# SaurabhIndi/unet-segmentation

Measured on AMD Instinct MI355X. Metric: training images/sec (512×512×1, batch=8) at 1/2/4/8 MI355X; IoU vs ref, higher is better.
Workload: dtype fp32; 1 GPU; U-Net train step 512x512x1, batch 8/GPU, fp32 GEMMs (fwd+WCE+bwd+SGD); global_batch=8, image=512, parallelism=dp1

## Files before the change

include/unet_hip.h:

```cpp
#ifndef UNET_HIP_H
#define UNET_HIP_H

#include <stddef.h>
#include <stdint.h>

#ifdef __cplusplus
extern "C" {
#endif

typedef void* unet_stream_t;

const char* unet_version(void);
const char* unet_last_error(void);

typedef struct unet_plan unet_plan;

unet_plan* unet_plan_create(int n, int c_in, int h, int w, int n_classes);

enum { UNET_PREC_FP32 = 0, UNET_PREC_BF16 = 1, UNET_PREC_BF16X3 = 2 };
unet_plan* unet_plan_create_ex(int n, int c_in, int h, int w, int n_classes, int precision);
int unet_plan_precision(const unet_plan* p);
void unet_plan_destroy(unet_plan* p);
int unet_plan_out_hw(const unet_plan* p, int* out_h, int* out_w);
size_t unet_plan_workspace_bytes(const unet_plan* p);
// ... 72 lines not shown
size_t unet_instance_masks_ws_bytes(int n, int h, int w);
int unet_instance_masks(const uint8_t* mask, int n, int h, int w, int min_size, uint16_t* labels, void* ws,
                        unet_stream_t stream);
size_t unet_rand_index_ws_bytes(int h, int w);
int unet_rand_index(const uint16_t* gt, const uint16_t* pred, int h, int w, double* out, void* ws,
                    unet_stream_t stream);

typedef struct unet_tracker unet_tracker;
unet_tracker* unet_tracker_create(int h, int w, double iou_track, double iou_division, int max_children);
void unet_tracker_destroy(unet_tracker* t);
size_t unet_tracker_ws_bytes(int h, int w);
int unet_tracker_add_frame(unet_tracker* t, const uint16_t* labels, int frame, void* ws, unet_stream_t stream);
int unet_tracker_step_host(unet_tracker* t, int frame, int n_curr, const int32_t* host_labels,
                           const int64_t* host_areas, const int64_t* host_inter);
int unet_tracker_num_tracks(const unet_tracker* t);
int unet_tracker_tracks(const unet_tracker* t, int32_t* host_out, int cap);
int unet_linear_sum_assignment(long long nr, long long nc, const double* host_cost, int64_t* host_row_ind,
                               int64_t* host_col_ind);

enum { UNET_CTC_SEG = 0, UNET_CTC_TRA = 1 };
enum { UNET_CTC_GT = 0, UNET_CTC_RES = 1 };
typedef struct unet_ctc unet_ctc;
unet_ctc* unet_ctc_create(void);
void unet_ctc_destroy(unet_ctc* c);
size_t unet_ctc_ws_bytes(int t, int h, int w);
int unet_ctc_add_frames(unet_ctc* c, int kind, const uint16_t* gt, const uint16_t* res, const int32_t* host_frames,
                        int t, int h, int w, void* ws, unet_stream_t stream);
int unet_ctc_add_frame_host(unet_ctc* c, int kind, int frame, int n_gt, const int32_t* host_gt_labels,
                            const int64_t* host_gt_areas, int n_res, const int32_t* host_res_labels,
                            const int64_t* host_res_areas, int n_pairs, const int64_t* host_pairs);
int unet_ctc_set_tracks(unet_ctc* c, int side, const int32_t* host_rows, int n);
int unet_ctc_measures(unet_ctc* c, double* host_out, int64_t* host_counts);
long long unet_ctc_log(unet_ctc* c, char* buf, size_t cap);
int unet_ctc_num_frames(const unet_ctc* c, int kind);
int unet_ctc_frame_sizes(const unet_ctc* c, int kind, int index, int32_t* host_out);
int unet_ctc_frame_tables(const unet_ctc* c, int kind, int index, int32_t* host_gt_labels, int64_t* host_gt_areas,
                          int32_t* host_res_labels, int64_t* host_res_areas, int64_t* host_pairs);
int unet_ctc_stats(const unet_ctc* c, int64_t* host_out);

enum { UNET_WARP_FORCE_WS = 1 };
size_t unet_warping_error_ws_bytes(int n, int h, int w);
int unet_warping_error(const uint16_t* gt, const uint8_t* pred, int n, int h, int w, int radius, int separate,
                       int max_sweeps, int flags, uint8_t* warped, int64_t* counts, void* ws, unet_stream_t stream);
void unet_simple_point_table(uint8_t out[256]);

int unet_set_tuning(const char* key, int value);
size_t unet_tuning_report(char* buf, size_t len);
int unet_tuning_reset(void);
long long unet_slab_fallbacks(int reset);
long long unet_nondeterministic_sites(int reset);
long long unet_fused_bnb_sites(int reset);
long long unet_wgrad_oihw_sites(int reset);
long long unet_igemm_plane_launches(int reset);
int unet_tuning_save(const char* path);
int unet_tuning_load(const char* path);

int unet_conv3x3_fwd(const float* x, int n, int h, int w, int ci, const float* wt_oihw,
                     const float* bias, int co, const float* x_scale, const float* x_shift,
                     float* y, void* ws, unet_stream_t stream);
int unet_conv3x3_dgrad(const float* dy, int n, int h, int w, int ci, const float* wt_oihw,
                       int co, float* dx, void* ws, unet_stream_t stream);
int unet_conv3x3_wgrad(const float* x, const float* dy, int n, int h, int w, int ci, int co,
                       float* dw_oihw, float* db, void* ws, unet_stream_t stream);
size_t unet_conv_ws_bytes(int n, int h, int w, int ci, int co);
int unet_convT2_fwd(const float* x, int n, int h, int w, int ci, const float* wt, const float* bias,
                    int co, float* y, void* ws, unet_stream_t stream);
int unet_convT2_bwd(const float* x, const float* dy, int n, int h, int w, int ci, const float* wt,
                    int co, float* dx, float* dw, float* db, void* ws, unet_stream_t stream);
int unet_maxpool2_fwd(const float* x, int n, int h, int w, int c, float* y, uint8_t* arg,
                      unet_stream_t stream);
int unet_maxpool2_bwd(const float* dy, const uint8_t* arg, int n, int h, int w, int c, float* dx,
                      unet_stream_t stream);
int unet_bn_train_fwd(const float* x, int n, int h, int w, int c, const float* gamma,
                      const float* beta, float* running_mean, float* running_var, float* y,
                      float* save_mean, float* save_invstd, void* ws, unet_stream_t stream);
int unet_bn_train_bwd(const float* x, const float* dy, int n, int h, int w, int c,
                      const float* gamma, const float* save_mean, const float* save_invstd,
                      float* dx, float* dgamma, float* dbeta, void* ws, unet_stream_t stream);
size_t unet_bn_ws_bytes(int c);

size_t unet_bn_relu_ws_bytes(int n, int h, int w, int c);
int unet_bn_relu_fwd(const float* x, int n, int h, int w, int c, const float* gamma, const float* beta,
                     float* running_mean, float* running_var, int64_t* nbt, float momentum, float eps,
                     int training, int relu, float* y, float* save_mean, float* save_invstd, void* ws,
                     unet_stream_t stream);
int unet_bn_relu_bwd(const float* x, const float* y, const float* dy, int n, int h, int w, int c,
                     const float* gamma, const float* save_mean, const float* save_invstd, int training,
                     int relu, float* dx, float* dgamma, float* dbeta, void* ws, unet_stream_t stream);
size_t unet_conv_first_ws_bytes(int n, int ci, int h, int w);
int unet_conv_first_fwd(const float* x_nchw, int n, int ci, int h, int w, const float* wt, const float* bias,
                        float* y, unet_stream_t stream);
int unet_conv_first_bwd(const float* x_nchw, const float* dy, int n, int ci, int h, int w, const float* wt,
                        float* dx_nchw, float* dw, float* db, void* ws, unet_stream_t stream);
size_t unet_conv1x1_ws_bytes(int k);
int unet_conv1x1_fwd(const float* x, int n, int h, int w, int c, const float* wt, const float* bias, int k,
                     float* logits_nchw, unet_stream_t stream);
int unet_conv1x1_bwd(const float* x, const float* dlogits_nchw, int n, int h, int w, int c, const float* wt, int k,
                     float* dx, float* dw, float* db, void* ws, unet_stream_t stream);

int unet_peak_probe(int kind, int reps, double* result, unet_stream_t stream);

#ifdef __cplusplus
}
#endif
#endif
```

unet-segmentation_amd/csrc/ops.hip:

```cpp
#include <algorithm>
#include <cerrno>
#include <string>

#include "../../include/unet_hip.h"
#include "unet_internal.h"

using namespace unet;

namespace unet {
extern int g_tune_igemm, g_tune_wgrad, g_autotune, g_force_split, g_force_tile, g_concurrent, g_wino_max,
    g_wino_dgrad_max, g_wino_wgrad_max, g_bf16_norm, g_bn_fold, g_wino4_fwd_min_cg, g_wino4_fwd_small_cg,
    g_maxpool_vec8, g_wgrad_fwd_u, g_ctc_chunk_frames, g_ctc_dense_cells;
hipError_t launch_fill(float* p, size_t n, float v, hipStream_t s);
hipError_t launch_pair_sum(const double* st, int g, int c, float* out, hipStream_t s);
}

namespace {
thread_local std::string g_op_err;
inline size_t al256(size_t b) { return (b + 255) / 256 * 256; }
int g_op_prec = UNET_PREC_FP32;
int g_op_a16 = 0;

hipError_t op_b_to_bf16(IgemmArgs& a, size_t n, void* scratch, hipStream_t s) {
  if (g_op_prec == UNET_PREC_FP32) return hipSuccess;
// ... 482 lines not shown
                     const int64_t* ts, const int64_t* wsd, float* loss, float* dl, float gscale, void* ws,
                     unet_stream_t st) {
  if (!ts || !wsd || k < 1) return -EINVAL;
  OPCK(launch_wce(logits, t, wm, n, k, h, w, ts, wsd, loss, dl, gscale, reinterpret_cast<double*>(ws),
                  reinterpret_cast<hipStream_t>(st)));
  return 0;
}

int unet_scale_by_device_scalar(float* x, size_t n, const float* g, unet_stream_t st) {
  OPCK(launch_scale_by_dev(x, x, n, g, reinterpret_cast<hipStream_t>(st)));
  return 0;
}

int unet_scale_by_device_scalar_out(const float* x, float* y, size_t n, const float* g, unet_stream_t st) {
  OPCK(launch_scale_by_dev(x, y, n, g, reinterpret_cast<hipStream_t>(st)));
  return 0;
}

int unet_sgd_momentum(float* p, const float* g, float* buf, size_t n, float lr, float mom, float gscale, int first,
                      unet_stream_t st) {
  OPCK(launch_sgd(p, g, buf, n, lr, mom, gscale, first, reinterpret_cast<hipStream_t>(st)));
  return 0;
}

int unet_iou_counts(const uint8_t* a, const uint8_t* b, size_t n, unsigned long long* out, unet_stream_t st) {
  OPCK(launch_iou(a, b, n, out, reinterpret_cast<hipStream_t>(st)));
  return 0;
}

int unet_set_tuning(const char* key, int value) {
  if (!key) return -EINVAL;
  const std::string k(key);
  if (k == "igemm_variant") g_tune_igemm = value;
  else if (k == "wgrad_variant") g_tune_wgrad = value;
  else if (k == "autotune") g_autotune = value;
  else if (k == "force_split") g_force_split = value;
  else if (k == "force_tile") g_force_tile = value;
  else if (k == "concurrent") g_concurrent = value;
  else if (k == "wino_max") g_wino_max = value;
  else if (k == "bf16_norm") g_bf16_norm = value;
  else if (k == "bn_fold") g_bn_fold = value != 0;
  else if (k == "wino_dgrad_max") g_wino_dgrad_max = value;
  else if (k == "wino_wgrad_max") g_wino_wgrad_max = value;
  else if (k == "wino4_fwd_min_cg") g_wino4_fwd_min_cg = value;
  else if (k == "wino4_fwd_small_cg") g_wino4_fwd_small_cg = value;
  else if (k == "op_a16") g_op_a16 = value != 0;
  else if (k == "maxpool_vec8") g_maxpool_vec8 = value;
  else if (k == "bnb_fuse") g_bnb_fuse = value;
  else if (k == "wgrad_early_u") g_wgrad_early_u = value;
  else if (k == "wgrad_fwd_u") g_wgrad_fwd_u = value;
  else if (k == "wgrad_plane") g_wgrad_plane = value;
  else if (k == "wgrad_oihw") g_wgrad_oihw = value;
  else if (k == "igemm_plane") g_igemm_plane = value;
  else if (k == "wino_point_tile") g_wino_point_tile = value;
  else if (k == "ctc_chunk_frames" || k == "ctc_dense_cells") {
    if (value < -1 || (value == 0 && k == "ctc_chunk_frames")) return -EINVAL;
    (k == "ctc_chunk_frames" ? g_ctc_chunk_frames : g_ctc_dense_cells) = value;
  }
  else if (k == "deterministic") g_deterministic = value != 0;
  else if (k == "op_precision") {
    if (value != UNET_PREC_FP32 && value != UNET_PREC_BF16 && value != UNET_PREC_BF16X3) return -EINVAL;
    g_op_prec = value;
  } else return -EINVAL;
  return 0;
}

int unet_tile_gather(const float* image, int c, int h, int w, int tile_in, int tile_out, int top, int left, int nx,
                     int first, int stride, int ntiles, float* tiles, unet_stream_t st) {
  if (!image || !tiles) return -EINVAL;
  OPCK(launch_tile_gather(image, c, h, w, tile_in, tile_out, top, left, nx, first, stride, ntiles, tiles,
                          reinterpret_cast<hipStream_t>(st)));
  return 0;
}

int unet_tile_scatter(const float* tile_logits, int k, int tile_out, int nx, int first, int stride, int ntiles, int h,
                      int w, float* logits, uint8_t* mask, unet_stream_t st) {
  if (!tile_logits) return -EINVAL;
  OPCK(launch_tile_scatter(tile_logits, k, tile_out, nx, first, stride, ntiles, h, w, logits, mask,
                           reinterpret_cast<hipStream_t>(st)));
  return 0;
}

size_t unet_instance_masks_ws_bytes(int n, int h, int w) {
  return n > 0 && h > 0 && w > 0 ? instance_masks_ws_bytes(n, h, w) : 0;
}

int unet_instance_masks(const uint8_t* mask, int n, int h, int w, int min_size, uint16_t* labels, void* ws,
                        unet_stream_t st) {
  if (!mask || !labels || !ws) return -EINVAL;
  OPCK(launch_instance_masks(mask, n, h, w, min_size, labels, ws, reinterpret_cast<hipStream_t>(st)));
  return 0;
}

size_t unet_rand_index_ws_bytes(int h, int w) { return h > 0 && w > 0 ? rand_index_ws_bytes(h, w) : 0; }

int unet_rand_index(const uint16_t* gt, const uint16_t* pred, int h, int w, double* out, void* ws,
                    unet_stream_t st) {
  if (!gt || !pred || !out || !ws) return -EINVAL;
  OPCK(launch_rand_index(gt, pred, h, w, out, ws, reinterpret_cast<hipStream_t>(st)));
  return 0;
}

size_t unet_weight_map_ws_bytes(int n) { return n > 0 ? weight_map_ws_bytes(n) : 0; }

int unet_weight_map(const uint16_t* labels, int n, int h, int w, double w0, double sigma, float* weights,
                    double* weights64, void* ws, unet_stream_t st) {
// ... 51 lines not shown
```

unet-segmentation_amd/csrc/plan.hip:

```cpp
#include <cerrno>
#include <cstdio>
#include <cstdlib>
#include <cstring>
#include <algorithm>
#include <array>
#include <map>
#include <mutex>
#include <string>
#include <vector>

#include "../../include/unet_hip.h"
#include "unet_internal.h"

using namespace unet;

namespace unet {
extern int g_wino_max, g_wino_dgrad_max, g_wino_wgrad_max, g_wino4_fwd_min_cg, g_wino4_fwd_small_cg;
int g_autotune = getenv("UNET_AUTOTUNE") ? atoi(getenv("UNET_AUTOTUNE")) : 1;
int g_concurrent = getenv("UNET_CONCURRENT") ? atoi(getenv("UNET_CONCURRENT")) : 1;
int g_bf16_norm = getenv("UNET_BF16_NORM") ? atoi(getenv("UNET_BF16_NORM")) : 0;
int g_bn_fold = getenv("UNET_BN_FOLD") ? atoi(getenv("UNET_BN_FOLD")) : 1;
int g_force_split = 0;
int g_force_tile = 0;
int g_deterministic = getenv("UNET_DETERMINISTIC") ? atoi(getenv("UNET_DETERMINISTIC")) : 0;
// ... 1327 lines not shown
  CK(launch_conv_first_dgrad(dy0, p->n, p->cin, p->h, p->w, P<float>(prm, L.pw), dx, s));
  return 0;
}

int unet_plan_wait_segment(unet_plan* p, int seg, unet_stream_t stream) {
  if (!p || seg < 0 || seg >= 9) {
    set_err("unet_plan_wait_segment: bad argument");
    return -EINVAL;
  }
  if (!p->seg_on_side[seg] || !p->side) return 0;
  CK(hipStreamWaitEvent(reinterpret_cast<hipStream_t>(stream), p->ev_seg[seg], 0));
  return 0;
}

int unet_plan_join(unet_plan* p, unet_stream_t stream) {
  if (!p) {
    set_err("unet_plan_join: null plan");
    return -EINVAL;
  }
  if (!p->side || !p->side_pending) return 0;
  CK(hipEventRecord(p->ev_join, p->side));
  CK(hipStreamWaitEvent(reinterpret_cast<hipStream_t>(stream), p->ev_join, 0));
  p->side_pending = false;
  return 0;
}

size_t unet_tuning_report(char* buf, size_t len) {
  std::string r;
  {
    std::lock_guard<std::mutex> lk(g_tune_mu);
    for (const auto& kv : g_tune_log) r += kv.second + "\n";
  }
  if (buf && len > 0) {
    const size_t k = std::min(len - 1, r.size());
    memcpy(buf, r.data(), k);
    buf[k] = 0;
  }
  return r.size() + 1;
}

long long unet_nondeterministic_sites(int reset) {
  return reset ? g_nondet_sites.exchange(0) : g_nondet_sites.load();
}

long long unet_fused_bnb_sites(int reset) {
  return reset ? unet::g_fused_bnb_sites.exchange(0) : unet::g_fused_bnb_sites.load();
}
long long unet_wgrad_oihw_sites(int reset) {
  return reset ? unet::g_wgrad_oihw_sites.exchange(0) : unet::g_wgrad_oihw_sites.load();
}
long long unet_igemm_plane_launches(int reset) {
  return reset ? unet::g_igemm_plane_launches.exchange(0) : unet::g_igemm_plane_launches.load();
}
long long unet_slab_fallbacks(int reset) {
  return reset ? g_slab_fallbacks.exchange(0) : g_slab_fallbacks.load();
}

int unet_tuning_reset(void) {
  std::lock_guard<std::mutex> lk(g_tune_mu);
  g_tuned.clear();
  g_tune_log.clear();
  return 0;
}

int unet_tuning_save(const char* path) {
  if (!path) return -EINVAL;
  std::lock_guard<std::mutex> lk(g_tune_mu);
  FILE* f = fopen(path, "w");
  if (!f) return -errno;
  for (const auto& kv : g_tuned) fprintf(f, "%s\t%d\t%d\n", kv.first.c_str(), kv.second.tile, kv.second.split);
  fclose(f);
  return (int)g_tuned.size();
}

int unet_tuning_load(const char* path) {
  if (!path) return -EINVAL;
  std::lock_guard<std::mutex> lk(g_tune_mu);
  return tune_db_read(path, true);
}

int unet_plan_set_timing(unet_plan* p, int enable) {
  if (!p) return -EINVAL;
  p->timing = enable != 0;
  return 0;
}

int unet_plan_timing(const unet_plan* pc, double* ms, double* fl, double* by, int* cnt) {
  auto* p = const_cast<unet_plan*>(pc);
  if (!p) return -EINVAL;
  int rc = 0;
  for (auto& e : p->evs) {
    float t = 0;
    if (hipEventSynchronize(e.b) != hipSuccess || hipEventElapsedTime(&t, e.a, e.b) != hipSuccess) {
      set_err("unet_plan_timing: event query failed");
      rc = -EIO;
    } else {
      p->t_ms[e.cls] += t;
      p->t_fl[e.cls] += e.flops;
      p->t_by[e.cls] += e.bytes;
      p->t_xf[e.cls] += e.xflops;
      p->t_n[e.cls] += 1;
      if (e.site >= 0) {
        auto& v = p->sites[e.site];
        v[0] += t;
        v[1] += e.flops;
        v[2] += e.xflops;
// ... 45 lines not shown
```

unet-segmentation_amd/csrc/unet_internal.h:

```cpp
#pragma once
#include <hip/hip_runtime.h>
#include <cstddef>
#include <cstdint>
#include <atomic>
#include <string>
#include <vector>

namespace unet {

constexpr int kMaxInChannels = 4096;
constexpr int kMaxClassCount = 4096;

struct Src {
  const float* ptr = nullptr;
  int H = 0, W = 0, C = 0;
  int oy = 0, ox = 0;
  const float* scale = nullptr;
  const float* shift = nullptr;
  int h16 = 0;
};

struct Gather {
  Src s[2];
  int c_split = 0;
// ... 6 lines not shown

struct Dst {
  float* ptr = nullptr;
  int H = 0, W = 0, C = 0;
  int oy = 0, ox = 0;
  int h16 = 0;
};

struct Epilogue {
  const float* bias = nullptr;
  int shuffle_co = 0;
  Dst d[2];
  int n_split = 1 << 30;
  int relu = 0;
  double* stats = nullptr;
  const float* yref = nullptr;
  int yref_h16 = 0;
  const float* bn_scale = nullptr;
  const float* bn_shift = nullptr;
  const float* bn_mean = nullptr;
  const float* bn_invstd = nullptr;
  double* bstats = nullptr;
  double* colsum1 = nullptr;
};

constexpr int kStatGroups = 64;

struct IgemmArgs {
  Gather a;
  const float* b = nullptr;
  const uint16_t* bh = nullptr;
  const uint16_t* bl = nullptr;
  int M, N, K;
  Epilogue e;
  int ksplit = 1;
  float* slab = nullptr;
  float* wino_ws = nullptr;
  size_t wino_ws_bytes = 0;
  int batch = 1;
  int batch_rows = 0;
  long long batch_b = 0;
  struct { int tile = -1, split = 1; } wino_choice;
  int fwd = 0;
};

extern std::atomic<long long> g_slab_fallbacks;
extern int g_deterministic;
extern int g_bnb_fuse;
extern int g_wgrad_early_u;
extern int g_wgrad_plane;
extern int g_wgrad_oihw;
extern int g_igemm_plane;
extern std::atomic<long long> g_igemm_plane_launches;
extern int g_wino_point_tile;
extern std::atomic<long long> g_nondet_sites;

struct WgradArgs {
  Gather ga;
  Gather gb;
  int Mo, No;
  int P;
  int pix_per_split;
  float* out;
  float* out_oihw = nullptr;
  float* slab = nullptr;
  size_t slab_bytes = 0;
  int accumulate = 0;
  int bf16 = 0;
  int split = 0;
  int batch = 1;
  long long batch_a = 0, batch_b = 0, batch_out = 0;
  float* wino_ws = nullptr;
  size_t wino_ws_bytes = 0;
  const float* vd_pre = nullptr;
  int u_ready = 0;
  int abl = 0;
};

struct GemmChoice {
  int tile = -1;
  int split = 1;
};

enum class IgemmFamily {
  Reg,
  Halo,
  Conv3Dma,
  Ring,
  Flat,
  C64,
  GemmRing,
  Wino,
  WinoFused
};
struct IgemmTile {
  int id;
  IgemmFamily family;
  int bm, bn, bk, slots;
  int th, tw, ch;
  int wino_m;
  bool bf16;
  bool x3;
  bool ksplit;
  bool tuned;
  bool (*fits)(const IgemmArgs&, const IgemmTile&);
  hipError_t (*go)(const IgemmArgs&, hipStream_t);
// ... 223 lines not shown
```

unet-segmentation_amd/csrc/winograd.hip:

```cpp
#include <algorithm>
#include <cstdlib>

#include "gemm_common.h"
#include "ring_common.h"

namespace unet {

__global__ void k_wino_w(const float* __restrict__ b, int N, int Cg, float* __restrict__ v) {
  const long long i = blockIdx.x * (long long)blockDim.x + threadIdx.x;
  if (i >= (long long)N * Cg) return;
  const int n = (int)(i / Cg), c = (int)(i - (long long)n * Cg);
  float g[3][3];
#pragma unroll
  for (int t = 0; t < 9; ++t) g[t / 3][t % 3] = b[((size_t)n * 9 + t) * Cg + c];
  float tg[4][3];
#pragma unroll
  for (int k = 0; k < 3; ++k) {
    tg[0][k] = g[0][k];
    tg[1][k] = 0.5f * (g[0][k] + g[1][k] + g[2][k]);
    tg[2][k] = 0.5f * (g[0][k] - g[1][k] + g[2][k]);
    tg[3][k] = g[2][k];
  }
  const size_t plane = (size_t)N * Cg, o = (size_t)n * Cg + c;
#pragma unroll
// ... 1511 lines not shown
      acc[p] = __builtin_amdgcn_mfma_f32_16x16x4f32(b.y, a.y, acc[p], 0, 0, 0);
    }
    lgkm_wait0();
    raw_barrier();
    issue_v(kn, 1);
  }
  vm_wait<0>();
  __syncthreads();
  wf64_output(acc, g, e, N, T, Th, Tw, t0, n0, th, cb, mi, mq, lane, wave, lds);
}

bool wino_fused64p_applies(const IgemmArgs& a) { return wino_fused64_applies(a) && a.a.Cg <= kWf64pMaxCg; }

hipError_t launch_wino_fused64p(const IgemmArgs& a, hipStream_t s) {
  if (!wino_fused64p_applies(a)) return hipErrorInvalidValue;
  const Gather& g = a.a;
  const int Th = (g.Hg + 3) / 4, Tw = (g.Wg + 3) / 4;
  const long long T = (long long)g.nimg * Th * Tw;
  float* V = reinterpret_cast<float*>(a.wino_ws);
  const long long nw = (long long)a.N * g.Cg;
  const int NB = a.N / 64;
  const long long G = (T + 31) / 32 * NB;
  hipLaunchKernelGGL(k_wino4f_w8, dim3((unsigned)((nw + 255) / 256)), dim3(256), 0, s, a.b, a.N, g.Cg, V);
  hipLaunchKernelGGL(k_wino4f64p, dim3((unsigned)G), dim3(512), 0, s, g, (const float*)V, a.N, T, Th, Tw, NB, a.e);
  return hipGetLastError();
}

__global__ void k_wino2f_w8(const float* __restrict__ b, int N, int Cg, float* __restrict__ v) {
  const long long i = blockIdx.x * (long long)blockDim.x + threadIdx.x;
  if (i >= (long long)N * Cg) return;
  const int n = (int)(i / Cg), c = (int)(i - (long long)n * Cg);
  float g[3][3];
#pragma unroll
  for (int t = 0; t < 9; ++t) g[t / 3][t % 3] = b[((size_t)n * 9 + t) * Cg + c];
  float tg[4][3];
#pragma unroll
  for (int k = 0; k < 3; ++k) {
    tg[0][k] = g[0][k];
    tg[1][k] = 0.5f * (g[0][k] + g[1][k] + g[2][k]);
    tg[2][k] = 0.5f * (g[0][k] - g[1][k] + g[2][k]);
    tg[3][k] = g[2][k];
  }
  const size_t base = (size_t)(c >> 3) * 16 * N;
  const int pos = wf8_slot(n, c & 3) + ((c >> 2) & 1);
#pragma unroll
  for (int r = 0; r < 4; ++r) {
    const float w4[4] = {tg[r][0], 0.5f * (tg[r][0] + tg[r][1] + tg[r][2]), 0.5f * (tg[r][0] - tg[r][1] + tg[r][2]),
                         tg[r][2]};
#pragma unroll
    for (int q = 0; q < 4; ++q) v[(base + (size_t)(r * 4 + q) * N + n) * 8 + pos] = w4[q];
  }
}

template <int NC>
__global__ __launch_bounds__(512, NC == 32 ? 2 : 1) void k_wino2f64(Gather g, const float* __restrict__ V, int N,
                                                                   long long T, int Th, int Tw, int NB, Epilogue e) {
  constexpr int TT = 64;
  constexpr int PU = TT * 8;
  constexpr int PV = NC * 8;
  constexpr int NJ = NC / 32;
  __shared__ __attribute__((aligned(16))) float lds[16 * PU + 16 * PV];
  float* Us = lds;
  float* Vs = lds + 16 * PU;
  const int tid = threadIdx.x, lane = tid & 63, wave = tid >> 6;
  long long bid = blockIdx.x;
  const long long G = gridDim.x;
  if ((G & 7) == 0) bid = (bid & 7) * (G >> 3) + (bid >> 3);
  const int nb = (int)(bid % NB);
  const long long t0 = (bid / NB) * TT;
  const int n0 = nb * NC;

  const int lt = tid >> 3, lc = tid & 7;
  const long long t = t0 + lt;
  int img = 0, ty = 0, tx = 0;
  if (t < T) {
    tx = (int)(t % Tw);
    const long long r = t / Tw;
    ty = (int)(r % Th);
    img = (int)(r / Th);
  }
  const int vrows = t < T ? min(4, g.Hg + 2 - 2 * ty) : 0;
  const int vcols = t < T ? min(4, g.Wg + 2 - 2 * tx) : 0;
  const bool wfull = __all(vrows == 4 && vcols == 4);
  float* const ubase = Us + lt * 8 + wf8_slot(lt, lc & 3) + (lc >> 2);
  float raw[16];
  float sc = 1.f, sh = 0.f;
  const int nk = g.Cg >> 3;
  const unsigned long long vbase = uniform_u64(V);
  const unsigned vlds = (unsigned)(size_t)(lds_u8_t*)lds + (unsigned)(16 * PU * 4);
  auto load = [&](int kc) {
    const bool second = kc * 8 >= g.c_split;
    const float* sp = second ? g.s[1].ptr : g.s[0].ptr;
    const int sH = second ? g.s[1].H : g.s[0].H, sW = second ? g.s[1].W : g.s[0].W;
    const int sC = second ? g.s[1].C : g.s[0].C;
    const int soy = second ? g.s[1].oy : g.s[0].oy, sox = second ? g.s[1].ox : g.s[0].ox;
    const int cl = kc * 8 - (second ? g.c_split : 0) + lc;
    const float* scp = second ? g.s[1].scale : g.s[0].scale;
    if (scp) {
      sc = scp[cl];
      sh = (second ? g.s[1].shift : g.s[0].shift)[cl];
    }
    const char* sb = reinterpret_cast<const char*>(sp);
    const unsigned o0 = ((unsigned)((img * sH + 2 * ty + soy) * sW + 2 * tx + sox) * sC + cl) * 4u;
    const unsigned rs = (unsigned)sW * sC * 4u, cs = (unsigned)sC * 4u;
    if (wfull) {
#pragma unroll
      for (int yy = 0; yy < 4; ++yy)
#pragma unroll
        for (int xx = 0; xx < 4; ++xx)
          raw[yy * 4 + xx] = *reinterpret_cast<const float*>(sb + (o0 + (yy * rs + xx * cs)));
    } else {
      const unsigned lr = (unsigned)max(vrows - 1, 0), lcn = (unsigned)max(vcols - 1, 0);
#pragma unroll
      for (int yy = 0; yy < 4; ++yy)
#pragma unroll
        for (int xx = 0; xx < 4; ++xx)
          raw[yy * 4 + xx] = *reinterpret_cast<const float*>(
              sb + (o0 + (min((unsigned)yy, lr) * rs + min((unsigned)xx, lcn) * cs)));
    }
  };
  auto commit = [&](int kc) {
    const bool second = kc * 8 >= g.c_split;
    const float* scp = second ? g.s[1].scale : g.s[0].scale;
    __builtin_amdgcn_s_waitcnt(0x0F70);
#pragma unroll
    for (int j = 0; j < 2 * NJ; ++j) {
      const int pc = wave + 8 * j;
      dma_sv((unsigned)((((size_t)kc * 16 + pc / NJ) * N + n0) * 32) + (unsigned)((pc % NJ) * 1024 + lane * 16),
             vbase, vlds + (unsigned)((pc / NJ) * PV * 4 + (pc % NJ) * 1024));
    }
    if (scp) {
#pragma unroll
      for (int q = 0; q < 16; ++q) raw[q] = fmaxf(fmaf(raw[q], sc, sh), 0.f);
    }
    if (!wfull) {
#pragma unroll
      for (int q = 0; q < 16; ++q) raw[q] = (q / 4 < vrows && q % 4 < vcols) ? raw[q] : 0.f;
    }
    float ev[4][4];
#pragma unroll
    for (int xx = 0; xx < 4; ++xx) {
      ev[0][xx] = raw[0 * 4 + xx] - raw[2 * 4 + xx];
      ev[1][xx] = raw[1 * 4 + xx] + raw[2 * 4 + xx];
      ev[2][xx] = raw[2 * 4 + xx] - raw[1 * 4 + xx];
      ev[3][xx] = raw[1 * 4 + xx] - raw[3 * 4 + xx];
    }
#pragma unroll
    for (int a = 0; a < 4; ++a) {
      ubase[(a * 4 + 0) * PU] = ev[a][0] - ev[a][2];
      ubase[(a * 4 + 1) * PU] = ev[a][1] + ev[a][2];
      ubase[(a * 4 + 2) * PU] = ev[a][2] - ev[a][1];
      ubase[(a * 4 + 3) * PU] = ev[a][1] - ev[a][3];
    }
    vm_wait<0>();
  };

  const int th = wave & 3, ch = wave >> 2;
  const int mi = lane & 15, mq = lane >> 4;
  const int aoff = (16 * th + mi) * 8 + wf8_slot(16 * th + mi, mq);
  const int boff = (16 * NJ * ch + mi) * 8 + wf8_slot(mi, mq);
  floatx4 acc[16][NJ];
#pragma unroll
  for (int p = 0; p < 16; ++p)
#pragma unroll
    for (int j = 0; j < NJ; ++j) acc[p][j] = (floatx4){0.f, 0.f, 0.f, 0.f};
  load(0);
  for (int kc = 0; kc < nk; ++kc) {
    commit(kc);
    __syncthreads();
    if (kc + 1 < nk) load(kc + 1);
#pragma unroll
    for (int p = 0; p < 16; ++p) {
      const float2 a = *reinterpret_cast<const float2*>(Us + p * PU + aoff);
#pragma unroll
      for (int j = 0; j < NJ; ++j) {
        const float2 b = *reinterpret_cast<const float2*>(Vs + p * PV + boff + 16 * j * 8);
        acc[p][j] = __builtin_amdgcn_mfma_f32_16x16x4f32(b.x, a.x, acc[p][j], 0, 0, 0);
        acc[p][j] = __builtin_amdgcn_mfma_f32_16x16x4f32(b.y, a.y, acc[p][j], 0, 0, 0);
      }
    }
    __syncthreads();
  }

  const long long tt = t0 + 16 * th + mi;
  const bool want = e.stats || e.yref || e.colsum1;
  const int nsplit = e.n_split < N ? e.n_split : N;
  const int grp = blockIdx.x % kStatGroups;
#pragma unroll
  for (int j = 0; j < NJ; ++j) {
    const int col0 = n0 + 16 * NJ * ch + 16 * j + 4 * mq;
    const bool second = col0 >= e.n_split;
    float* dptr = second ? e.d[1].ptr : e.d[0].ptr;
    const int dC = second ? e.d[1].C : e.d[0].C;
    const int dcol = second ? col0 - e.n_split : col0;
    const bool bwd_mask = e.yref != nullptr && !second;
    const float4 bias = e.bias ? ld4(e.bias + col0) : make_float4(0.f, 0.f, 0.f, 0.f);
    float4 bsc = make_float4(0.f, 0.f, 0.f, 0.f), bsh = bsc, bmu = bsc, bis = bsc;
    if (bwd_mask) { bsc = ld4(e.bn_scale + col0); bsh = ld4(e.bn_shift + col0); bmu = ld4(e.bn_mean + col0); bis = ld4(e.bn_invstd + col0); }
    float s1[4] = {0.f, 0.f, 0.f, 0.f}, s2[4] = {0.f, 0.f, 0.f, 0.f};
    if (tt < T) {
      const int ox = (int)(tt % Tw);
      const long long rq = tt / Tw;
      const int oy = (int)(rq % Th), on = (int)(rq / Th);
      float4 y4[4];
      if (bwd_mask) {
#pragma unroll
        for (int a = 0; a < 2; ++a)
#pragma unroll
          for (int bb = 0; bb < 2; ++bb) {
            const int y = min(2 * oy + a, g.Hg - 1), x = min(2 * ox + bb, g.Wg - 1);
            y4[a * 2 + bb] = ld4(e.yref + ((size_t)(on * g.Hg + y) * g.Wg + x) * dC + dcol);
          }
      }
      __builtin_amdgcn_s_waitcnt(0x0F70);
      float o[4][2][2];
#pragma unroll
      for (int r = 0; r < 4; ++r) {
        float w[2][4];
#pragma unroll
        for (int xx = 0; xx < 4; ++xx) {
          const float m0 = acc[0 * 4 + xx][j][r], m1 = acc[1 * 4 + xx][j][r];
          const float m2 = acc[2 * 4 + xx][j][r], m3 = acc[3 * 4 + xx][j][r];
          w[0][xx] = m0 + m1 + m2;
          w[1][xx] = m1 - m2 - m3;
        }
#pragma unroll
        for (int a = 0; a < 2; ++a) {
          o[r][a][0] = w[a][0] + w[a][1] + w[a][2];
          o[r][a][1] = w[a][1] - w[a][2] - w[a][3];
        }
      }
      const float bsv[4] = {bias.x, bias.y, bias.z, bias.w};
      const float scv[4] = {bsc.x, bsc.y, bsc.z, bsc.w}, shv[4] = {bsh.x, bsh.y, bsh.z, bsh.w};
      const float muv[4] = {bmu.x, bmu.y, bmu.z, bmu.w}, isv[4] = {bis.x, bis.y, bis.z, bis.w};
#pragma unroll
      for (int a = 0; a < 2; ++a) {
        const int y = 2 * oy + a;
        if (y >= g.Hg) continue;
#pragma unroll
        for (int bb = 0; bb < 2; ++bb) {
          const int x = 2 * ox + bb;
          if (x >= g.Wg) continue;
          const size_t idx = ((size_t)(on * g.Hg + y) * g.Wg + x) * dC + dcol;
          const float4 yq = bwd_mask ? y4[a * 2 + bb] : make_float4(0.f, 0.f, 0.f, 0.f);
          const float yv[4] = {yq.x, yq.y, yq.z, yq.w};
          float v[4];
#pragma unroll
          for (int r = 0; r < 4; ++r) v[r] = wf_epi(o[r][a][bb] + bsv[r], yv[r], scv[r], shv[r], muv[r], isv[r],
                                                     bwd_mask, e.relu, s1[r], s2[r]);
          st4(dptr + idx, make_float4(v[0], v[1], v[2], v[3]));
        }
      }
    }
    if (!want) continue;
#pragma unroll
    for (int r = 0; r < 4; ++r)
#pragma unroll
      for (int o2 = 1; o2 < 16; o2 <<= 1) {
        s1[r] += __shfl_xor(s1[r], o2);
        s2[r] += __shfl_xor(s2[r], o2);
      }
    if (mi == 0) {
#pragma unroll
      for (int r = 0; r < 4; ++r) {
        const int col = col0 + r;
        if (col < nsplit) {
          double* st = e.yref ? e.bstats : e.stats;
          if (st) {
            atomicAdd(st + ((size_t)grp * nsplit + col) * 2 + 0, (double)s1[r]);
            atomicAdd(st + ((size_t)grp * nsplit + col) * 2 + 1, (double)s2[r]);
          }
        } else if (e.colsum1) {
          atomicAdd(e.colsum1 + (size_t)grp * (N - nsplit) + (col - nsplit), (double)s1[r]);
        }
      }
    }
  }
}

bool wino_fused2_applies(const IgemmArgs& a, int nc) {
  const Gather& g = a.a;
  if (a.b == nullptr || a.bh != nullptr || a.batch != 1) return false;
  if (g.taps_h != 3 || g.taps_w != 3 || g.stride != 1 || a.K != 9 * g.Cg || g.Cg % 8 != 0 || g.c_split % 8 != 0 ||
      a.N % nc != 0 || (a.e.n_split < a.N && a.e.n_split % 16 != 0))
    return false;
  if (g.s[0].h16 || g.s[1].h16 || a.e.shuffle_co || a.e.d[0].h16 || a.e.d[1].h16 || a.e.yref_h16) return false;
  if (a.e.d[0].oy || a.e.d[0].ox || a.e.d[0].H != g.Hg || a.e.d[0].W != g.Wg) return false;
  if (a.e.n_split < a.N && (a.e.d[1].oy || a.e.d[1].ox || a.e.d[1].H != g.Hg || a.e.d[1].W != g.Wg)) return false;
  for (int k = 0; k < 2; ++k)
    if ((long long)g.nimg * g.s[k].H * g.s[k].W * g.s[k].C * 4 >= (1ll << 32)) return false;
  const long long T = (long long)g.nimg * ((g.Hg + 1) / 2) * ((g.Wg + 1) / 2);
  if ((T + 63) / 64 * (a.N / nc) > 0x7fffffffLL) return false;
  return a.wino_ws != nullptr && (size_t)16 * a.N * g.Cg * 4 <= a.wino_ws_bytes;
}

hipError_t launch_wino_fused2(const IgemmArgs& a, hipStream_t s, int nc) {
  if ((nc != 64 && nc != 32) || !wino_fused2_applies(a, nc)) return hipErrorInvalidValue;
  const Gather& g = a.a;
  const int Th = (g.Hg + 1) / 2, Tw = (g.Wg + 1) / 2;
  const long long T = (long long)g.nimg * Th * Tw;
  float* V = reinterpret_cast<float*>(a.wino_ws);
  const long long nw = (long long)a.N * g.Cg;
  const int NB = a.N / nc;
  const long long G = (T + 63) / 64 * NB;
  hipLaunchKernelGGL(k_wino2f_w8, dim3((unsigned)((nw + 255) / 256)), dim3(256), 0, s, a.b, a.N, g.Cg, V);
  if (nc == 64)
    hipLaunchKernelGGL(k_wino2f64<64>, dim3((unsigned)G), dim3(512), 0, s, g, (const float*)V, a.N, T, Th, Tw, NB, a.e);
  else
    hipLaunchKernelGGL(k_wino2f64<32>, dim3((unsigned)G), dim3(512), 0, s, g, (const float*)V, a.N, T, Th, Tw, NB, a.e);
  return hipGetLastError();
}

__device__ __forceinline__ void a6(const float (&y)[4], float (&r)[6]) {
  r[0] = y[0];
  r[1] = y[0] + y[1] + y[2] + y[3];
  r[2] = y[0] - y[1] + y[2] - y[3];
  r[3] = y[0] + 2.f * y[1] + 4.f * y[2] + 8.f * y[3];
  r[4] = y[0] - 0.5f * y[1] + 0.25f * y[2] - 0.125f * y[3];
  r[5] = y[3];
}
__device__ __forceinline__ void gt3(const float (&m)[6], float (&r)[3]) {
  r[0] = m[0] + (m[2] - m[1]) * (1.f / 3.f) + (m[3] - 16.f * m[4]) * (1.f / 15.f);
  r[1] = -(m[1] + m[2]) * (1.f / 3.f) + (2.f * m[3] + 8.f * m[4]) * (1.f / 15.f);
  r[2] = (m[2] - m[1]) * (1.f / 3.f) + (4.f * m[3] - 4.f * m[4]) * (1.f / 15.f) + m[5];
}

__global__ __launch_bounds__(256) void k_wino4_dy(Src dy, int Hg, int Wg, int Th, int Tw, long long T, int Co,
                                                  float* __restrict__ vd) {
  const long long i = blockIdx.x * (long long)blockDim.x + threadIdx.x;
  if (i >= T * Co) return;
  const long long t = i / Co;
  const int c = (int)(i - t * Co);
  const int tx = (int)(t % Tw);
  const long long r = t / Tw;
  const int ty = (int)(r % Th), n = (int)(r / Th);
  float e[6][4];
#pragma unroll
  for (int xx = 0; xx < 4; ++xx) {
    float d[4];
#pragma unroll
    for (int yy = 0; yy < 4; ++yy) {
      const int y = 4 * ty + yy, x = 4 * tx + xx;
      const bool in = y < Hg && x < Wg;
      const float v = dy.ptr[((size_t)(n * dy.H + (in ? y : 0) + dy.oy) * dy.W + (in ? x : 0) + dy.ox) * dy.C + c];
      d[yy] = in ? v : 0.f;
    }
    float rr[6];
    a6(d, rr);
#pragma unroll
    for (int a = 0; a < 6; ++a) e[a][xx] = rr[a];
  }
  const size_t plane = (size_t)T * Co, o = (size_t)t * Co + c;
#pragma unroll
  for (int a = 0; a < 6; ++a) {
    float rr[6];
    a6(e[a], rr);
#pragma unroll
    for (int bb = 0; bb < 6; ++bb) vd[(a * 6 + bb) * plane + o] = rr[bb];
  }
}

__device__ __forceinline__ void wout_store(const float (&dwv)[9], long long i, long long n, int Ci,
// ... 400 lines not shown
```

unet-segmentation_amd/unet_amd/_lib.py:

```python
from __future__ import annotations

import ctypes
import os

_HERE = os.path.dirname(os.path.abspath(__file__))
LIB_PATH = os.environ.get("UNET_HIP_LIB", os.path.join(_HERE, "libunet_hip.so"))

_vp = ctypes.c_void_p
_i = ctypes.c_int
_f = ctypes.c_float
_sz = ctypes.c_size_t

SIGNATURES = {
    "unet_version": (ctypes.c_char_p, []),
    "unet_last_error": (ctypes.c_char_p, []),
    "unet_plan_create": (_vp, [_i, _i, _i, _i, _i]),
    "unet_plan_create_ex": (_vp, [_i, _i, _i, _i, _i, _i]),
    "unet_plan_precision": (_i, [_vp]),
    "unet_plan_destroy": (None, [_vp]),
    "unet_plan_out_hw": (_i, [_vp, ctypes.POINTER(_i), ctypes.POINTER(_i)]),
    "unet_plan_workspace_bytes": (_sz, [_vp]),
    "unet_plan_forward_workspace_bytes": (_sz, [_vp]),
    "unet_plan_num_params": (_i, [_vp]),
    "unet_plan_num_grads": (_i, [_vp]),
# ... 34 lines not shown
    "unet_conv3x3_fwd": (_i, [_vp, _i, _i, _i, _i, _vp, _vp, _i, _vp, _vp, _vp, _vp, _vp]),
    "unet_conv3x3_dgrad": (_i, [_vp, _i, _i, _i, _i, _vp, _i, _vp, _vp, _vp]),
    "unet_conv3x3_wgrad": (_i, [_vp, _vp, _i, _i, _i, _i, _i, _vp, _vp, _vp, _vp]),
    "unet_conv_ws_bytes": (_sz, [_i, _i, _i, _i, _i]),
    "unet_convT2_fwd": (_i, [_vp, _i, _i, _i, _i, _vp, _vp, _i, _vp, _vp, _vp]),
    "unet_convT2_bwd": (_i, [_vp, _vp, _i, _i, _i, _i, _vp, _i, _vp, _vp, _vp, _vp, _vp]),
    "unet_maxpool2_fwd": (_i, [_vp, _i, _i, _i, _i, _vp, _vp, _vp]),
    "unet_maxpool2_bwd": (_i, [_vp, _vp, _i, _i, _i, _i, _vp, _vp]),
    "unet_bn_train_fwd": (_i, [_vp, _i, _i, _i, _i, _vp, _vp, _vp, _vp, _vp, _vp, _vp, _vp, _vp]),
    "unet_bn_train_bwd": (_i, [_vp, _vp, _i, _i, _i, _i, _vp, _vp, _vp, _vp, _vp, _vp, _vp, _vp]),
    "unet_bn_ws_bytes": (_sz, [_i]),
    "unet_bn_relu_ws_bytes": (_sz, [_i, _i, _i, _i]),
    "unet_bn_relu_fwd": (_i, [_vp, _i, _i, _i, _i, _vp, _vp, _vp, _vp, _vp, _f, _f, _i, _i, _vp, _vp, _vp, _vp,
                              _vp]),
    "unet_bn_relu_bwd": (_i, [_vp, _vp, _vp, _i, _i, _i, _i, _vp, _vp, _vp, _i, _i, _vp, _vp, _vp, _vp, _vp]),
    "unet_conv_first_ws_bytes": (_sz, [_i, _i, _i, _i]),
    "unet_conv_first_fwd": (_i, [_vp, _i, _i, _i, _i, _vp, _vp, _vp, _vp]),
    "unet_conv_first_bwd": (_i, [_vp, _vp, _i, _i, _i, _i, _vp, _vp, _vp, _vp, _vp, _vp]),
    "unet_conv1x1_ws_bytes": (_sz, [_i]),
    "unet_conv1x1_fwd": (_i, [_vp, _i, _i, _i, _i, _vp, _vp, _i, _vp, _vp]),
    "unet_conv1x1_bwd": (_i, [_vp, _vp, _i, _i, _i, _i, _vp, _i, _vp, _vp, _vp, _vp, _vp]),
    "unet_peak_probe": (_i, [_i, _i, ctypes.POINTER(ctypes.c_double), _vp]),
    "unet_tracker_create": (_vp, [_i, _i, ctypes.c_double, ctypes.c_double, _i]),
    "unet_tracker_destroy": (None, [_vp]),
    "unet_tracker_ws_bytes": (_sz, [_i, _i]),
    "unet_tracker_add_frame": (_i, [_vp, _vp, _i, _vp, _vp]),
    "unet_tracker_step_host": (_i, [_vp, _i, _i, _vp, _vp, _vp]),
    "unet_tracker_num_tracks": (_i, [_vp]),
    "unet_tracker_tracks": (_i, [_vp, _vp, _i]),
    "unet_linear_sum_assignment": (_i, [ctypes.c_longlong, ctypes.c_longlong, _vp, _vp, _vp]),
    "unet_ctc_create": (_vp, []),
    "unet_ctc_destroy": (None, [_vp]),
    "unet_ctc_ws_bytes": (_sz, [_i, _i, _i]),
    "unet_ctc_add_frames": (_i, [_vp, _i, _vp, _vp, _vp, _i, _i, _i, _vp, _vp]),
    "unet_ctc_add_frame_host": (_i, [_vp, _i, _i, _i, _vp, _vp, _i, _vp, _vp, _i, _vp]),
    "unet_ctc_set_tracks": (_i, [_vp, _i, _vp, _i]),
    "unet_ctc_measures": (_i, [_vp, _vp, _vp]),
    "unet_ctc_log": (ctypes.c_longlong, [_vp, ctypes.c_char_p, _sz]),
    "unet_ctc_num_frames": (_i, [_vp, _i]),
    "unet_ctc_frame_sizes": (_i, [_vp, _i, _i, _vp]),
    "unet_ctc_frame_tables": (_i, [_vp, _i, _i, _vp, _vp, _vp, _vp, _vp]),
    "unet_ctc_stats": (_i, [_vp, _vp]),
    "unet_warping_error_ws_bytes": (_sz, [_i, _i, _i]),
    "unet_warping_error": (_i, [_vp, _vp, _i, _i, _i, _i, _i, _i, _i, _vp, _vp, _vp, _vp]),
    "unet_simple_point_table": (None, [_vp]),
    "unet_set_tuning": (_i, [ctypes.c_char_p, _i]),
    "unet_tuning_report": (_sz, [ctypes.c_char_p, _sz]),
    "unet_tuning_reset": (_i, []),
    "unet_slab_fallbacks": (ctypes.c_longlong, [_i]),
    "unet_nondeterministic_sites": (ctypes.c_longlong, [_i]),
    "unet_fused_bnb_sites": (ctypes.c_longlong, [_i]),
    "unet_wgrad_oihw_sites": (ctypes.c_longlong, [_i]),
    "unet_igemm_plane_launches": (ctypes.c_longlong, [_i]),
    "unet_tuning_save": (_i, [ctypes.c_char_p]),
    "unet_tuning_load": (_i, [ctypes.c_char_p]),
}

_lib = None
_load_error = None


def load():
    global _lib, _load_error
    if _lib is not None:
        return _lib
    if _load_error is not None:
        raise RuntimeError(_load_error)
    try:
        lib = ctypes.CDLL(LIB_PATH, mode=ctypes.RTLD_GLOBAL)
    except OSError as e:
        _load_error = (f"libunet_hip.so could not be loaded from {LIB_PATH} ({e}); "
                       "build it with `python -c 'import __graft_entry__ as g; g.build()'`")
        raise RuntimeError(_load_error) from e
    for name, (res, args) in SIGNATURES.items():
        fn = getattr(lib, name)
        fn.restype = res
        fn.argtypes = args
    _lib = lib
    return lib


def last_error() -> str:
    msg = load().unet_last_error()
    return msg.decode() if msg else ""


def check(rc: int, what: str) -> None:
    if rc != 0:
        raise RuntimeError(f"{what} failed (rc={rc}): {last_error()}")


def ptr(t) -> int:
    return None if t is None else t.data_ptr()


def ptr_array(tensors):
    arr = (ctypes.c_void_p * len(tensors))()
    for i, t in enumerate(tensors):
        arr[i] = t.data_ptr()
    return arr


def stream_of(device=None):
    import torch
    return ctypes.c_void_p(torch.cuda.current_stream(device).cuda_stream)

# ... 37 lines not shown
```

Before: 317.4 images/s.

## Double-buffer LDS in fused Winograd F2 kernel with wave-specialized pipelining

Adds a pipelined variant of the fused Winograd F(2,3) MFMA kernel for NC=64. It uses two U and two V LDS buffers, so the input transform and the V DMA for the next channel chunk overlap with the MFMA work on the current chunk. Half the waves commit early and half commit after their MFMAs, which replaces the two per-iteration __syncthreads with a single raw barrier. The cost is doubled LDS use (lower occupancy headroom) plus more complex vmcnt accounting, which could race if the counts are wrong. It is on by default behind an env toggle.

```diff
diff --git a/include/unet_hip.h b/include/unet_hip.h
--- a/include/unet_hip.h
+++ b/include/unet_hip.h
@@ -148,6 +148,7 @@
 long long unet_fused_bnb_sites(int reset);
 long long unet_wgrad_oihw_sites(int reset);
 long long unet_igemm_plane_launches(int reset);
+long long unet_wino_fused_pipe_launches(int reset);
 int unet_tuning_save(const char* path);
 int unet_tuning_load(const char* path);
 
diff --git a/unet-segmentation_amd/csrc/ops.hip b/unet-segmentation_amd/csrc/ops.hip
--- a/unet-segmentation_amd/csrc/ops.hip
+++ b/unet-segmentation_amd/csrc/ops.hip
@@ -558,6 +558,7 @@
   else if (k == "wgrad_plane") g_wgrad_plane = value;
   else if (k == "wgrad_oihw") g_wgrad_oihw = value;
   else if (k == "igemm_plane") g_igemm_plane = value;
+  else if (k == "wino_fused_pipe") g_wino_fused_pipe = value;
   else if (k == "wino_point_tile") g_wino_point_tile = value;
   else if (k == "ctc_chunk_frames" || k == "ctc_dense_cells") {
     if (value < -1 || (value == 0 && k == "ctc_chunk_frames")) return -EINVAL;
diff --git a/unet-segmentation_amd/csrc/plan.hip b/unet-segmentation_amd/csrc/plan.hip
--- a/unet-segmentation_amd/csrc/plan.hip
+++ b/unet-segmentation_amd/csrc/plan.hip
@@ -1403,6 +1403,9 @@
 long long unet_igemm_plane_launches(int reset) {
   return reset ? unet::g_igemm_plane_launches.exchange(0) : unet::g_igemm_plane_launches.load();
 }
+long long unet_wino_fused_pipe_launches(int reset) {
+  return reset ? unet::g_wino_fused_pipe_launches.exchange(0) : unet::g_wino_fused_pipe_launches.load();
+}
 long long unet_slab_fallbacks(int reset) {
   return reset ? g_slab_fallbacks.exchange(0) : g_slab_fallbacks.load();
 }
diff --git a/unet-segmentation_amd/csrc/unet_internal.h b/unet-segmentation_amd/csrc/unet_internal.h
--- a/unet-segmentation_amd/csrc/unet_internal.h
+++ b/unet-segmentation_amd/csrc/unet_internal.h
@@ -82,6 +82,8 @@
 extern int g_wgrad_oihw;
 extern int g_igemm_plane;
 extern std::atomic<long long> g_igemm_plane_launches;
+extern int g_wino_fused_pipe;
+extern std::atomic<long long> g_wino_fused_pipe_launches;
 extern int g_wino_point_tile;
 extern std::atomic<long long> g_nondet_sites;
 
diff --git a/unet-segmentation_amd/csrc/winograd.hip b/unet-segmentation_amd/csrc/winograd.hip
--- a/unet-segmentation_amd/csrc/winograd.hip
+++ b/unet-segmentation_amd/csrc/winograd.hip
@@ -1587,16 +1587,18 @@
   }
 }
 
-template <int NC>
+template <int NC, bool PIPE>
 __global__ __launch_bounds__(512, NC == 32 ? 2 : 1) void k_wino2f64(Gather g, const float* __restrict__ V, int N,
                                                                    long long T, int Th, int Tw, int NB, Epilogue e) {
   constexpr int TT = 64;
   constexpr int PU = TT * 8;
   constexpr int PV = NC * 8;
   constexpr int NJ = NC / 32;
-  __shared__ __attribute__((aligned(16))) float lds[16 * PU + 16 * PV];
+  static_assert(!PIPE || NC == 64, "the pipelined loop needs two U and two V buffers");
+  constexpr int NU = PIPE ? 2 : 1;
+  __shared__ __attribute__((aligned(16))) float lds[NU * 16 * PU + NU * 16 * PV];
   float* Us = lds;
-  float* Vs = lds + 16 * PU;
+  float* Vs = lds + NU * 16 * PU;
   const int tid = threadIdx.x, lane = tid & 63, wave = tid >> 6;
   long long bid = blockIdx.x;
   const long long G = gridDim.x;
@@ -1622,7 +1624,7 @@
   float sc = 1.f, sh = 0.f;
   const int nk = g.Cg >> 3;
   const unsigned long long vbase = uniform_u64(V);
-  const unsigned vlds = (unsigned)(size_t)(lds_u8_t*)lds + (unsigned)(16 * PU * 4);
+  const unsigned vlds = (unsigned)(size_t)(lds_u8_t*)lds + (unsigned)(NU * 16 * PU * 4);
   auto load = [&](int kc) {
     const bool second = kc * 8 >= g.c_split;
     const float* sp = second ? g.s[1].ptr : g.s[0].ptr;
@@ -1654,16 +1656,20 @@
               sb + (o0 + (min((unsigned)yy, lr) * rs + min((unsigned)xx, lcn) * cs)));
     }
   };
-  auto commit = [&](int kc) {
+  auto issue_v = [&](int kc, int buf) {
+#pragma unroll
+    for (int j = 0; j < 2 * NJ; ++j) {
+      const int pc = wave + 8 * j;
+      dma_sv((unsigned)((((size_t)kc * 16 + pc / NJ) * N + n0) * 32) + (unsigned)((pc % NJ) * 1024 + lane * 16),
+             vbase, vlds + (unsigned)(buf * 16 * PV * 4 + (pc / NJ) * PV * 4 + (pc % NJ) * 1024));
+    }
+  };
+  auto commit = [&](int kc, int ub, int vb, bool vfirst) {
     const bool second = kc * 8 >= g.c_split;
     const float* scp = second ? g.s[1].scale : g.s[0].scale;
     __builtin_amdgcn_s_waitcnt(0x0F70);
-#pragma unroll
-    for (int j = 0; j < 2 * NJ; ++j) {
-      const int pc = wave + 8 * j;
-      dma_sv((unsigned)((((size_t)kc * 16 + pc / NJ) * N + n0) * 32) + (unsigned)((pc % NJ) * 1024 + lane * 16),
-             vbase, vlds + (unsigned)((pc / NJ) * PV * 4 + (pc % NJ) * 1024));
-    }
+    if (vfirst) issue_v(kc, vb);
+    float* const ub_ = ubase + ub * 16 * PU;
     if (scp) {
 #pragma unroll
       for (int q = 0; q < 16; ++q) raw[q] = fmaxf(fmaf(raw[q], sc, sh), 0.f);
@@ -1682,12 +1688,11 @@
     }
 #pragma unroll
     for (int a = 0; a < 4; ++a) {
-      ubase[(a * 4 + 0) * PU] = ev[a][0] - ev[a][2];
-      ubase[(a * 4 + 1) * PU] = ev[a][1] + ev[a][2];
-      ubase[(a * 4 + 2) * PU] = ev[a][2] - ev[a][1];
-      ubase[(a * 4 + 3) * PU] = ev[a][1] - ev[a][3];
-    }
-    vm_wait<0>();
+      ub_[(a * 4 + 0) * PU] = ev[a][0] - ev[a][2];
+      ub_[(a * 4 + 1) * PU] = ev[a][1] + ev[a][2];
+      ub_[(a * 4 + 2) * PU] = ev[a][2] - ev[a][1];
+      ub_[(a * 4 + 3) * PU] = ev[a][1] - ev[a][3];
+    }
   };
 
   const int th = wave & 3, ch = wave >> 2;
@@ -1699,22 +1704,61 @@
   for (int p = 0; p < 16; ++p)
 #pragma unroll
     for (int j = 0; j < NJ; ++j) acc[p][j] = (floatx4){0.f, 0.f, 0.f, 0.f};
-  load(0);
-  for (int kc = 0; kc < nk; ++kc) {
-    commit(kc);
-    __syncthreads();
-    if (kc + 1 < nk) load(kc + 1);
+  auto mfma = [&](int ub, int vb) {
+    const float* const Uc = Us + ub * 16 * PU + aoff;
+    const float* const Vc = Vs + vb * 16 * PV + boff;
 #pragma unroll
     for (int p = 0; p < 16; ++p) {
-      const float2 a = *reinterpret_cast<const float2*>(Us + p * PU + aoff);
+      const float2 a = *reinterpret_cast<const float2*>(Uc + p * PU);
 #pragma unroll
       for (int j = 0; j < NJ; ++j) {
-        const float2 b = *reinterpret_cast<const float2*>(Vs + p * PV + boff + 16 * j * 8);
+        const float2 b = *reinterpret_cast<const float2*>(Vc + p * PV + 16 * j * 8);
         acc[p][j] = __builtin_amdgcn_mfma_f32_16x16x4f32(b.x, a.x, acc[p][j], 0, 0, 0);
         acc[p][j] = __builtin_amdgcn_mfma_f32_16x16x4f32(b.y, a.y, acc[p][j], 0, 0, 0);
       }
     }
-    __syncthreads();
+  };
+  load(0);
+  if constexpr (!PIPE) {
+    for (int kc = 0; kc < nk; ++kc) {
+      commit(kc, 0, 0, true);
+      vm_wait<0>();
+      __syncthreads();
+      if (kc + 1 < nk) load(kc + 1);
+      mfma(0, 0);
+      __syncthreads();
+    }
+  } else {
+    auto wait_v = [&](int kc) {
+      if (kc >= nk) vm_wait<0>();
+      else if ((kc * 8 >= g.c_split ? g.s[1].scale : g.s[0].scale) != nullptr) vm_wait<18>();
+      else vm_wait<16>();
+      lgkm_wait0();
+      raw_barrier();
+    };
+    const bool late = __builtin_amdgcn_readfirstlane(wave) >= 4;
+    commit(0, 0, 0, true);
+    if (nk > 1) load(1);
+    wait_v(1);
+    for (int kc = 0; kc < nk; ++kc) {
+      const bool more = kc + 1 < nk;
+      const int cb = kc & 1;
+      if (more) {
+        if (late) {
+          commit(kc + 1, cb ^ 1, cb ^ 1, true);
+          if (kc + 2 < nk) load(kc + 2);
+        } else {
+          issue_v(kc + 1, cb ^ 1);
+        }
+      }
+      mfma(cb, cb);
+      if (!more) break;
+      if (!late) {
+        commit(kc + 1, cb ^ 1, cb ^ 1, false);
+        if (kc + 2 < nk) load(kc + 2);
+      }
+      wait_v(kc + 2);
+    }
   }
 
   const long long tt = t0 + 16 * th + mi;
@@ -1813,6 +1857,9 @@
   }
 }
 
+int g_wino_fused_pipe = getenv("UNET_WINO_FUSED_PIPE") ? atoi(getenv("UNET_WINO_FUSED_PIPE")) : 1;
+std::atomic<long long> g_wino_fused_pipe_launches{0};
+
 bool wino_fused2_applies(const IgemmArgs& a, int nc) {
   const Gather& g = a.a;
   if (a.b == nullptr || a.bh != nullptr || a.batch != 1) return false;
@@ -1839,10 +1886,14 @@
   const int NB = a.N / nc;
   const long long G = (T + 63) / 64 * NB;
   hipLaunchKernelGGL(k_wino2f_w8, dim3((unsigned)((nw + 255) / 256)), dim3(256), 0, s, a.b, a.N, g.Cg, V);
-  if (nc == 64)
-    hipLaunchKernelGGL(k_wino2f64<64>, dim3((unsigned)G), dim3(512), 0, s, g, (const float*)V, a.N, T, Th, Tw, NB, a.e);
-  else
-    hipLaunchKernelGGL(k_wino2f64<32>, dim3((unsigned)G), dim3(512), 0, s, g, (const float*)V, a.N, T, Th, Tw, NB, a.e);
+#define WF2(NC_, P_) \
+  hipLaunchKernelGGL((k_wino2f64<NC_, P_>), dim3((unsigned)G), dim3(512), 0, s, g, (const float*)V, a.N, T, Th, Tw, NB, a.e)
+  const bool pipe = nc == 64 && g_wino_fused_pipe != 0;
+  if (pipe) WF2(64, true);
+  else if (nc == 64) WF2(64, false);
+  else WF2(32, false);
+#undef WF2
+  if (pipe) ++g_wino_fused_pipe_launches;
   return hipGetLastError();
 }
 
diff --git a/unet-segmentation_amd/unet_amd/_lib.py b/unet-segmentation_amd/unet_amd/_lib.py
--- a/unet-segmentation_amd/unet_amd/_lib.py
+++ b/unet-segmentation_amd/unet_amd/_lib.py
@@ -110,6 +110,7 @@
     "unet_fused_bnb_sites": (ctypes.c_longlong, [_i]),
     "unet_wgrad_oihw_sites": (ctypes.c_longlong, [_i]),
     "unet_igemm_plane_launches": (ctypes.c_longlong, [_i]),
+    "unet_wino_fused_pipe_launches": (ctypes.c_longlong, [_i]),
     "unet_tuning_save": (_i, [ctypes.c_char_p]),
     "unet_tuning_load": (_i, [ctypes.c_char_p]),
 }
```

Result: no change. 319.5 images/s, median of 6 (+0.7%).
